# sarahappleby/VAMP

Hardware: AMD Instinct MI355X
Metric: walker-steps/sec (log-posterior evals/sec) (higher is better)
Workload: dtype f64

## Files before the change

### __graft_entry__.py

```python
import os
import subprocess
import sys

ROOT = os.path.dirname(os.path.abspath(__file__))
if ROOT not in sys.path:
    sys.path.insert(0, ROOT)


def build() -> None:
    from vamp_amd import build as vb
    vb.build()
    subprocess.check_call(["make", "-C", os.path.join(ROOT, "oracle"), "-s"])
    host = os.path.join(ROOT, "tests", "host")
    so = os.path.join(host, "libvoigt_host.so")
    src = os.path.join(host, "voigt_host.cpp")
    hdr = os.path.join(ROOT, "vamp_amd", "csrc", "voigt_math.hpp")
    if not os.path.exists(so) or os.path.getmtime(so) < max(os.path.getmtime(src), os.path.getmtime(hdr)):
        subprocess.check_call(["g++", "-O2", "-std=c++17", "-shared", "-fPIC", "-ffp-contract=off", "-o", so, src])
    pso, psrc = os.path.join(host, "libff_pred_host.so"), os.path.join(host, "ff_pred_host.cpp")
    phdr = os.path.join(ROOT, "vamp_amd", "csrc", "ff_predicates.hpp")
    if not os.path.exists(pso) or os.path.getmtime(pso) < max(os.path.getmtime(psrc), os.path.getmtime(phdr), os.path.getmtime(hdr)):
        subprocess.check_call(["g++", "-O2", "-std=c++17", "-shared", "-fPIC", "-ffp-contract=off", "-o", pso, psrc])
    oso, osrc = os.path.join(host, "libnp_order_host.so"), os.path.join(host, "np_order_host.cpp")
    if not os.path.exists(oso) or os.path.getmtime(oso) < max(os.path.getmtime(osrc), os.path.getmtime(phdr), os.path.getmtime(hdr)):
        subprocess.check_call(["g++", "-O2", "-std=c++17", "-shared", "-fPIC", "-ffp-contract=off", "-o", oso, osrc])
    sso, ssrc = os.path.join(host, "libsuper_nodes_host.so"), os.path.join(host, "super_nodes_host.cpp")
    sinc = os.path.join(ROOT, "vamp_amd", "csrc", "ff_super.inc")
    if not os.path.exists(sso) or os.path.getmtime(sso) < max(os.path.getmtime(ssrc), os.path.getmtime(phdr), os.path.getmtime(hdr), os.path.getmtime(sinc)):
        subprocess.check_call(["g++", "-O2", "-std=c++17", "-shared", "-fPIC", "-ffp-contract=off", "-o", sso, ssrc])
    gso, gsrc = os.path.join(host, "libvoigt_grad_host.so"), os.path.join(host, "voigt_grad_host.cpp")
    ghdr = os.path.join(ROOT, "vamp_amd", "csrc", "voigt_grad.hpp")
    if not os.path.exists(gso) or os.path.getmtime(gso) < max(os.path.getmtime(gsrc), os.path.getmtime(ghdr), os.path.getmtime(hdr)):
        subprocess.check_call(["g++", "-O2", "-std=c++17", "-shared", "-fPIC", "-ffp-contract=off", "-o", gso, gsrc])
    fake, fsrc = os.path.join(host, "librccl_fake.so"), os.path.join(host, "rccl_fake.cpp")
    if not os.path.exists(fake) or os.path.getmtime(fake) < os.path.getmtime(fsrc):
        subprocess.check_call([os.environ.get("HIPCC", "/opt/rocm/bin/hipcc"), "-O1", "-std=c++17", "-shared", "-fPIC", "-o", fake, fsrc, "-lrt"])
    import vamp_amd
    os.environ.setdefault("VAMP_NO_IMPORT_ORDER_WARNING", "1")
    vamp_amd._lib.load()


def smoke() -> None:
    import numpy as np
    import torch

    import vamp_amd
    from oracle import vamp_oracle as vo

    g = np.load(os.path.join(ROOT, "tests", "golden", "lnprob_cases.npz"), allow_pickle=False)
    name = "H1215_r0_K4_m1_sd0"
    x, f, n, th = g[name + "_x"], g[name + "_flux"], g[name + "_noise"], g[name + "_theta"]
    region = vo.Region(x=x, flux=f, noise=n, n_comp=4, mode=vo.MODE_VOIGT4)
# ... 44 lines not shown
```

### vamp_amd/csrc/ff_predicates.hpp

```cpp
#pragma once
#include "voigt_math.hpp"

namespace vamp {

constexpr double FF_ZONE_MARGIN = 1.0 / 1024.0;

VAMP_DEV bool ff_tile_in_zone(double c, double s, double y, double mid, double half) {
    const double Xf = (fabs(mid - c) + half) * s;
    return fma(Xf, Xf, y * y) < R2_CORE * (1.0 - FF_ZONE_MARGIN);
}

#ifndef VAMP_SUPER_DIST
#define VAMP_SUPER_DIST 4.0
#endif
#ifndef VAMP_FF_R2_M3
#define VAMP_FF_R2_M3 300.0
#endif
VAMP_DEV bool ff_super_distant(double c, double s, double y, double Mid, double Half) {
    const double distS = fabs(Mid - c) - Half;
    const double Xe = distS * s;
    return (distS >= VAMP_SUPER_DIST * Half) & (fma(Xe, Xe, y * y) >= VAMP_FF_R2_M3);
}
VAMP_DEV double ff_super_r2e(double c, double s, double y, double Mid, double Half) {
    const double Xe = (fabs(Mid - c) - Half) * s;
    return fma(Xe, Xe, y * y);
}
VAMP_DEV void ff_super_tile(double mid0, double half0, double mid3, double half3, double& Mid, double& Half) {
    const double lo = fmin(mid0 - half0, mid3 - half3), hi = fmax(mid0 + half0, mid3 + half3);
    Mid = 0.5 * (lo + hi);
    Half = 0.5 * (hi - lo);
}

struct SuperOrder {
    unsigned long long seq;
    int n, iters, iters3;
};
VAMP_DEV SuperOrder super_order(unsigned dist, unsigned d3) {
    SuperOrder o;
    const unsigned cls[2] = {d3 & dist, dist & ~d3};
    unsigned long long seq = 0ull;
    int sh = 0;
    for (int c = 0; c < 2; ++c)
        for (unsigned m = cls[c]; m; m &= m - 1u) {
            seq |= (unsigned long long)__builtin_ctz(m) << sh;
            sh += 4;
        }
    o.seq = seq;
    o.n = sh >> 2;
    o.iters = (o.n + 7) >> 3;
    o.iters3 = (__builtin_popcount(cls[0]) + 7) >> 3;
    return o;
}

// ... 29 lines not shown
```

### vamp_amd/csrc/vamp_hip.hip

```cpp
#include <hip/hip_runtime.h>
#include <dlfcn.h>

#include <algorithm>
#include <atomic>
#include <chrono>
#include <cmath>
#include <cstdint>
#include <cstdio>
#include <cstdlib>
#include <cstring>
#include <new>
#include <string>
#include <vector>

#include "../../include/vamp_hip.h"
#include "abi_state.hpp"
#include "draws.hpp"
#include "host_plan.hpp"
#include "map_search.hpp"
#include "voigt_math.hpp"
#include "ff_predicates.hpp"
#include "ff_moments.hpp"

#ifndef VAMP_EARLY_LOADS
// ... 50 lines not shown
#ifndef VAMP_MID_Z2
#define VAMP_MID_Z2 30.25
#endif
#ifndef VAMP_WIDE_MAX
#define VAMP_WIDE_MAX 0.75
#endif
#ifndef VAMP_F32_LEAN_STAGE
#define VAMP_F32_LEAN_STAGE 1
#endif
#ifndef VAMP_TILE_MOMENTS
#define VAMP_TILE_MOMENTS 2
#endif
#ifndef VAMP_NODE_PASS
#define VAMP_NODE_PASS 1
#endif
#ifndef VAMP_NP_CLASS_RUNS
#define VAMP_NP_CLASS_RUNS 1
#endif
#ifndef VAMP_DEAL_ADJ
#define VAMP_DEAL_ADJ 1
#endif
#ifndef VAMP_SUPER_NODES
#define VAMP_SUPER_NODES 1
#endif
#ifndef VAMP_TAB_PAIR
#define VAMP_TAB_PAIR 0
#endif
#ifndef VAMP_TILE_HEAD
#define VAMP_TILE_HEAD 0
#endif
namespace {

constexpr int KMAX = 16;
constexpr int KMAX_ALL = VAMP_MAX_COMPONENTS;
static_assert(KMAX_ALL >= KMAX && KMAX_ALL < 64, "lane k stages line k; one spare lane for sd");
constexpr int WAVES_PER_BLOCK = 4;
constexpr long long PACK_MIN_WALKERS = 16384;
constexpr int RES_MAX_MOVERS = 128;
#ifndef VAMP_RES_WAVES
#define VAMP_RES_WAVES 8
#endif
constexpr int RES_MAX_WAVES = VAMP_RES_WAVES;
constexpr int BLOCK = 64 * WAVES_PER_BLOCK;
constexpr int DMAX = 4 * KMAX_ALL + 1;
#ifndef VAMP_SPLIT_MAX_WALKERS
#define VAMP_SPLIT_MAX_WALKERS (1ll << 62)
// ... 956 lines not shown
            chi = fma(r, r, chi);
        }
    }
    }
}

#if VAMP_NODE_PASS && VAMP_TILE_MOMENTS != 1 && !VAMP_X_PREFETCH && !defined(VAMP_SKIP_NEAR) && !defined(VAMP_SKIP_FFNODES) && \
    !defined(VAMP_SKIP_CLENSHAW) && !defined(VAMP_SKIP_EXP)
#define VAMP_NODE_PASS_ON 1
#else
#define VAMP_NODE_PASS_ON 0
#endif
#if VAMP_NODE_PASS_ON
__device__ __forceinline__ unsigned ff_fold16(unsigned long long m) {
    const unsigned h = (unsigned)m | (unsigned)(m >> 32);
    return (h | (h >> 16)) & 0xffffu;
}
#if VAMP_SUPER_NODES && VAMP_DEAL_ADJ
#define VAMP_SUPER_ON 1
#include "ff_super.inc"
#else
#define VAMP_SUPER_ON 0
#endif
struct NodeSets { unsigned far, n6, n4, n3, wide; };
template <bool WIDE, bool ZONE, class LDS>
__device__ __forceinline__ void ff_classify_batch_np(const LDS& L, const double2* __restrict__ geo, int K, int lane_, int base, int stride,
                                                     unsigned wide_all, unsigned long long& farmasks, unsigned long long& widemasks,
                                                     unsigned long long& zonemasks, NodeSets& sets, double& mid, double& half) {
    int lane = lane_;
    asm volatile("" : "+v"(lane));
    const int j = lane >> 4, k = lane & (KMAX - 1);
    const double2 g = geo[(base + j * stride) >> 8];
    mid = g.x, half = fabs(g.y);
    const LineRec& me = *reinterpret_cast<const LineRec*>(reinterpret_cast<const char*>(L.line) +
                                                          __umul24((unsigned)(k < K ? k : 0), (unsigned)sizeof(LineRec)));
    const double my_c = me.c, my_s = me.s, my_y = me.y, my_w8 = me.w8, my_wmid = me.wmid;
    const double dist = fabs(mid - my_c) - half;
    const bool my_beyond = (k < K) & (dist >= FF_DIST * half);
    const bool my_far = my_beyond & (dist >= my_w8);
    const double Xe = dist * my_s, r2e = fma(Xe, Xe, my_y * my_y);
    farmasks = __ballot(my_far);
    sets.far = ff_fold16(farmasks);
    sets.n6 = ff_fold16(__ballot(my_far & (r2e < VAMP_FF_R2_M4)));
    sets.n4 = ff_fold16(__ballot(my_far & (r2e < VAMP_FF_R2_M3)));
    sets.n3 = ff_fold16(__ballot(my_far & (r2e < VAMP_FF_R2_M2)));
    widemasks = 0ull;
    if constexpr (WIDE) {
        const bool my_wide = ((((wide_all >> k) & 1u) != 0u) | (VAMP_MID_NODES && (my_beyond & (dist >= my_wmid)))) & !my_far;
        widemasks = __ballot(my_wide);
    }
    sets.wide = ff_fold16(widemasks);
    zonemasks = 0ull;
    if constexpr (ZONE) zonemasks = __ballot(vamp::ff_tile_in_zone(my_c, my_s, my_y, mid, half));
}
constexpr double FF_X_IDLE = 64.0;
static_assert(FF_X_IDLE * FF_X_IDLE >= VAMP_FF_R2_M2 && FF_X_IDLE < vamp::X_FAR, "the idle argument neither deepens a pair nor needs a guard");
template <int M> struct NpDepth { static constexpr int value = M; };
#if VAMP_SUPER_ON
template <class LDS>
__device__ __forceinline__ double ff_super_pass(const LDS& L, TileScratch& Sx, const double* __restrict__ dct, int lane, double xnode,
                                                unsigned dist, unsigned d3, double Mid, double Half) {
    const vamp::SuperOrder ord = vamp::super_order(dist, d3);
    const int n = lane & (FF_NODES - 1), g4 = (lane >> 4) * 4;
    const double xs = fma(Half, dct[FF_MAT + n], Mid);
    unsigned long long seq = ord.seq;
    int left = ord.n;
    double acc = 0.0;
    auto run = [&](auto depth, int iters) {
        constexpr int M = decltype(depth)::value;
#pragma unroll 1
        for (int i = 0; i < iters; ++i) {
            const unsigned s32 = (unsigned)seq >> g4;
            double X[2], y[2], amp[2], r2[2], nn[2], d[2];
#pragma unroll
            for (int t = 0; t < 2; ++t) {
                const LineRec& ln = *reinterpret_cast<const LineRec*>(reinterpret_cast<const char*>(L.line) +
                                                                      __umul24((s32 >> (16 * t)) & 15u, (unsigned)sizeof(LineRec)));
                const bool live = (g4 >> 2) + 4 * t < left;
                const double Xl = fabs(xs - ln.c) * ln.s;
                X[t] = live ? Xl : FF_X_IDLE;
                y[t] = ln.y;
                amp[t] = live ? ln.amp : 0.0;
                r2[t] = fma(X[t], X[t], y[t] * y[t]);
                vamp::voigt_jfrac_nd<M>(X[t], y[t], r2[t], nn[t], d[t], vamp::GHFrac<M>::Z, vamp::GHFrac<M>::C);
            }
            const double ra = vamp::rcp_nr(d[0] * d[1]);
            acc = fma(amp[0], nn[0] * (ra * d[1]), acc);
            acc = fma(amp[1], nn[1] * (ra * d[0]), acc);
            seq >>= 32;
            left -= 8;
        }
    };
    run(NpDepth<3>{}, ord.iters3);
    run(NpDepth<2>{}, ord.iters - ord.iters3);
    {
        const int me = lane_here();
        const int a16 = (me ^ 16) << 2, a32 = (me ^ 32) << 2;
        acc += __hiloint2double(__builtin_amdgcn_ds_bpermute(a16, __double2hiint(acc)), __builtin_amdgcn_ds_bpermute(a16, __double2loint(acc)));
        acc += __hiloint2double(__builtin_amdgcn_ds_bpermute(a32, __double2hiint(acc)), __builtin_amdgcn_ds_bpermute(a32, __double2loint(acc)));
    }
    if (lane < FF_NODES) Sx.coef[lane] = acc;
    __builtin_amdgcn_wave_barrier();
    const double2* crow = reinterpret_cast<const double2*>(FF_SUPER_C) + n;
    const double2* fv = reinterpret_cast<const double2*>(Sx.coef);
    double a0 = 0.0, a1 = 0.0;
#pragma unroll
    for (int n2 = 0; n2 < FF_NODES / 2; ++n2) {
        const double2 m = crow[n2 * FF_NODES], f2 = fv[n2];
        a0 = fma(m.x, f2.x, a0);
        a1 = fma(m.y, f2.y, a1);
    }
    __builtin_amdgcn_wave_barrier();
    if (lane < FF_NODES) Sx.coef[lane] = a0 + a1;
    __builtin_amdgcn_wave_barrier();
    const double t = (xnode - Mid) * vamp::rcp_nr(Half), t2 = t + t;
    double b1 = 0.0, b2 = 0.0;
#pragma unroll
    for (int k = FF_NODES - 1; k >= 1; --k) {
        const double b = fma(t2, b1, Sx.coef[k] - b2);
        b2 = b1;
        b1 = b;
    }
    const double p = fma(t, b1, Sx.coef[0] - b2);
    __builtin_amdgcn_wave_barrier();
    return p;
}
template <class LDS>
__device__ __forceinline__ double ff_super_batch(const LDS& L, TileScratch& Sx, const double* __restrict__ dct, const double2* __restrict__ geo,
                                                 int K, int lane_, int base, int stride, double mid, double half,
                                                 unsigned long long farmasks, NodeSets& sets) {
    int lane = lane_;
    asm volatile("" : "+v"(lane));
    const int k = lane & (KMAX - 1);
    const LineRec& me = *reinterpret_cast<const LineRec*>(reinterpret_cast<const char*>(L.line) +
                                                          __umul24((unsigned)(k < K ? k : 0), (unsigned)sizeof(LineRec)));
    const double my_c = me.c, my_s = me.s, my_y = me.y;
    const double2 g0 = geo[base >> 8], g3 = geo[(base + (FF_BATCH - 1) * stride) >> 8];
    double Mid, Half;
    vamp::ff_super_tile(g0.x, fabs(g0.y), g3.x, fabs(g3.y), Mid, Half);
    const bool my_dist = (k < K) & vamp::ff_super_distant(my_c, my_s, my_y, Mid, Half);
    const bool my_d3 = my_dist & (vamp::ff_super_r2e(my_c, my_s, my_y, Mid, Half) < VAMP_FF_R2_M2);
    const unsigned all4 = (unsigned)farmasks & (unsigned)(farmasks >> 16) & (unsigned)(farmasks >> 32) & (unsigned)(farmasks >> 48) & 0xffffu;
    const unsigned dist = (unsigned)__ballot(my_dist) & all4;
    if (dist == 0u) return 0.0;
    const unsigned d3 = (unsigned)__ballot(my_d3) & dist;
    sets.far &= ~dist, sets.n6 &= ~dist, sets.n4 &= ~dist, sets.n3 &= ~dist;
    const double xnode = fma(half, dct[FF_MAT + (lane & (FF_NODES - 1))], mid);
    return ff_super_pass(L, Sx, dct, lane, xnode, dist, d3, Mid, Half);
}
#endif
template <bool WIDE, bool GUARD, class LDS>
__device__ __forceinline__ double ff_node_pass(const LDS& L, const double* __restrict__ dct, const double* tab, int lane_, double mid, double half,
                                               unsigned long long farmasks, unsigned long long widemasks, NodeSets sets, double fs0 = 0.0) {
    int lane = lane_;
    asm volatile("" : "+v"(lane));
    const double xnode = fma(half, dct[FF_MAT + (lane & (FF_NODES - 1))], mid);
    double fs = fs0;
    const unsigned far16 = ff_tile_field(farmasks, lane);
#if VAMP_NP_CLASS_RUNS
    if (sets.far != 0u) {
    const vamp::NpOrder ord = vamp::np_pair_order(sets.far, sets.n6, sets.n4, sets.n3);
    unsigned long long seq = ord.seq;
    const unsigned far16b = far16 & ~ord.solo;
    struct Pair { double c[2], s[2], y[2], amp[2]; };
    auto read_pair = [&](unsigned long long q) {
        Pair p;
#pragma unroll
        for (int t = 0; t < 2; ++t) {
            const LineRec& ln = L.line[(unsigned)(q >> (4 * t)) & 15u];
            p.c[t] = ln.c, p.s[t] = ln.s, p.y[t] = ln.y, p.amp[t] = ln.amp;
        }
// ... 123 lines not shown
}
__device__ __forceinline__ void ff_moment_chi_nodes_row(TileScratch& Sx, const double* __restrict__ mt, int lane, int j, double a_row, double c0,
                                                        double& chi) {
    if ((lane >> 4) == j) Sx.coef[lane & (FF_NODES - 1)] = a_row;
    const int n = lane & (FF_NODES - 1), g4 = (lane >> 4) * 4;
    const double2* Qr = reinterpret_cast<const double2*>(mt + vamp::FFN_Q + n * FF_NODES + g4);
    const double2 q01 = Qr[0], q23 = Qr[1];
    const double Sv = mt[vamp::FFN_S + n];
    __builtin_amdgcn_wave_barrier();
    const double2* av = reinterpret_cast<const double2*>(Sx.coef + g4);
    const double2 a01 = av[0], a23 = av[1];
    const double a = Sx.coef[n];
    const double acc0 = fma(q01.x, a01.x, 0.5 * Sv), acc1 = q01.y * a01.y;
    const double term = a * (fma(q23.x, a23.x, acc0) + fma(q23.y, a23.y, acc1));
    chi += lane == 0 ? term + c0 : term;
    __builtin_amdgcn_wave_barrier();
}
template <int MODE, class PK, bool TAB, bool WIDE = false, bool GUARD = true, bool SUPER = false>
__device__ __forceinline__ void sweep_range_ff_np(const RegionDev& R, const typename PK::Lds& L, TileScratch& Sx, const double* __restrict__ dct,
                                                  const double* __restrict__ x, const double* __restrict__ f,
                                                  const double* __restrict__ wt, const double* __restrict__ ut,
                                                  const double2* __restrict__ geo, int lane, int base0, int base1, int stride,
                                                  double& chi, const double* tab, unsigned long long wide_all = 0ull,
                                                  const double* __restrict__ mom = nullptr) {
    constexpr int T = TPIX;
    static_assert(PK::LPW == 64 && PK::KCAP <= 16, "far-field tiles: one walker per wavefront, <= 16 lines");
    const int K = R.K;
    const int ntile = base0 < base1 ? (base1 - base0 + stride - 1) / stride : 0;
#if VAMP_DEAL_ADJ
    (void)ntile;
    const int tstride = 64 * T, bstep = FF_BATCH * stride;
    const int bfull = __builtin_amdgcn_readfirstlane((base1 / bstep) * bstep);
    const int bfirst = FF_BATCH * base0, brest = bfull + base0;
#else
    const int tstride = stride, bstep = FF_BATCH * stride;
    const int bfull = __builtin_amdgcn_readfirstlane(base0 + (ntile / FF_BATCH) * (FF_BATCH * stride));
    const int bfirst = base0, brest = bfull;
#endif
    for (int batch = __builtin_amdgcn_readfirstlane(bfirst); batch < bfull; batch += bstep) {
    unsigned long long farmasks, widemasks, zonemasks;
    double fsn;
    {
        NodeSets sets;
        double mid_j, half_j;
        ff_classify_batch_np<WIDE, TAB>(L, geo, K, lane, batch, tstride, (unsigned)wide_all, farmasks, widemasks, zonemasks, sets, mid_j, half_j);
#if VAMP_SUPER_ON
        double fs0 = 0.0;
        if constexpr (SUPER) {
            if (__builtin_amdgcn_readfirstlane((int)(unsigned)wide_all) == 0) {
                fs0 = ff_super_batch(L, Sx, dct, geo, K, lane, batch, tstride, mid_j, half_j, farmasks, sets);
            }
        }
        fsn = ff_node_pass<WIDE, GUARD>(L, dct, tab, lane, mid_j, half_j, farmasks, widemasks, sets, fs0);
#else
        fsn = ff_node_pass<WIDE, GUARD>(L, dct, tab, lane, mid_j, half_j, farmasks, widemasks, sets);
#endif
    }
#if VAMP_TILE_MOMENTS == 2
    {
        unsigned long long fm = farmasks, wm = widemasks;
        double a_row = 0.0, amax_row = 0.0;
        bool have_a = false;
#pragma unroll 1
        for (int j = 0; j < FF_BATCH; ++j, fm >>= KMAX, wm >>= KMAX) {
            const unsigned farmask = (unsigned)fm & 0xffffu, widemask = WIDE ? (unsigned)wm & 0xffffu : 0u;
            if ((~(farmask | widemask) & ((1u << K) - 1u)) != 0u) continue;
            const double* mt = mom + ((batch + j * tstride) >> 8) * MOM_TILE;
            const double root_c0 = mt[MOM_RC], root_q0 = mt[MOM_RQ];
            if (!vamp::ff_moments_try(root_c0, root_q0)) continue;
            if (!have_a) {
                int eoff = FF_EXP;
                asm volatile("" : "+s"(eoff));
                a_row = -vamp::expm1_taylor_tab(-fsn, dct + eoff);
// ... 314 lines not shown
#endif
#ifndef VAMP_SKIP_CLENSHAW
            ff32_horner<T>(Sx, u, up, tau);
#endif
        }
#pragma unroll
        for (int t = 0; t < T; ++t) {
            const int i = base + 64 * t + lane;
#ifdef VAMP_SKIP_EXP
            const float m = 1.0f - tau[t];
#else
            const float m = __expf(-tau[t]);
#endif
            const float r = (f[i] - m) * wt[i];
            chi += (double)r * (double)r;
        }
    }
    }
}

struct PixPtrs {
    const double* x; const double* f; const double* wt;
    const float* xf; const float* ff; const float* wtf;
    const double* u; const float* uf; const double2* geo;
    const double* mom;
};

template <bool F32>
__global__ __launch_bounds__(64 * TPIX) void k_tile_tables(const RegionDev* __restrict__ regions, const double* __restrict__ x,
                                                           const float* __restrict__ xf, double* __restrict__ u, float* __restrict__ uf,
                                                           double2* __restrict__ geo, const double* __restrict__ f = nullptr,
                                                           const double* __restrict__ wt = nullptr, double* __restrict__ mom = nullptr) {
    const RegionDev& R = regions[blockIdx.y];
    const int base = (int)blockIdx.x * (64 * TPIX), i = base + (int)threadIdx.x;
    if (i >= R.P) return;
    const long long g = R.pix_off + i;
    if (base + 64 * TPIX > R.P) {
        if constexpr (F32) uf[g] = 0.0f;
        else u[g] = 0.0;
        return;
    }
    const long long g0 = R.pix_off + base, g1 = g0 + 64 * TPIX - 1;
    const double x_lo = F32 ? (double)xf[g0] : x[g0], x_hi = F32 ? (double)xf[g1] : x[g1];
    const double mid = 0.5 * (x_lo + x_hi), half = 0.5 * fabs(x_hi - x_lo);
    const bool up = x_hi > x_lo;
    const int t = (int)threadIdx.x >> 6, q = up ? t : TPIX - 1 - t;
    double ug = 0.0;
    if constexpr (F32) {
        const float hf = (float)half, mf = (float)mid;
// ... 99 lines not shown
        if constexpr (VAMP_FARFIELD && PK::FF && MODE != VAMP_GAUSS3 && TPIX == 4)
            sweep_range_f32_ff<MODE, PK, use_tables32<F32, MODE, PK>()>(R, L, Sx, dct, x, f, wt, px.uf + R.pix_off, px.geo + (R.pix_off >> 8),
                                                                        lane, base0, full, stride, chi, reinterpret_cast<const float*>(tab));
        else if (TPIX > 1) sweep_range_f32<MODE, PK, TPIX>(R, L, x, f, wt, lane, base0, full, stride, chi);
        if constexpr (PK::TAIL || TPIX == 1)
            if (tail) {
                const int from = TPIX > 1 ? full : 0;
                if constexpr (!PK::FF && TPIX > 1) {
                    const int nt = (R.P - from + PK::LPW - 1) / PK::LPW;
                    if constexpr (TPIX >= 4) { if (nt == 4) sweep_range_f32<MODE, PK, 4>(R, L, x, f, wt, lane, from, from + 1, 1 << 28, chi); }
                    if constexpr (TPIX >= 3) { if (nt == 3) sweep_range_f32<MODE, PK, 3>(R, L, x, f, wt, lane, from, from + 1, 1 << 28, chi); }
                    if (nt == 2) sweep_range_f32<MODE, PK, 2>(R, L, x, f, wt, lane, from, from + 1, 1 << 28, chi);
                    else if (nt == 1) sweep_range_f32<MODE, PK, 1>(R, L, x, f, wt, lane, from, from + 1, 1 << 28, chi);
                } else {
                    sweep_range_f32<MODE, PK, 1>(R, L, x, f, wt, lane, from, R.P, PK::LPW, chi);
                }
            }
    } else {
        const double* x = px.x + R.pix_off; const double* f = px.f + R.pix_off; const double* wt = px.wt + R.pix_off;
        if constexpr (VAMP_FARFIELD && PK::FF && MODE != VAMP_GAUSS3 && TPIX == 4) {
            const double* ut = px.u + R.pix_off;
            const double2* geo = px.geo + (R.pix_off >> 8);
            const double* mom = VAMP_TILE_MOMENTS ? px.mom + (R.pix_off >> 8) * MOM_TILE : nullptr;
            const int flags = __builtin_amdgcn_readfirstlane((int)(__double_as_longlong(L.theta[4 * PK::KCAP + 2]) & 0x3ffff));
            const bool guard = (flags >> 16) != 0;
            if constexpr (VAMP_WIDE_NODES && TAB) {
                const unsigned long long wide_all = (unsigned long long)(flags & 0xffff);
                if (VAMP_MID_NODES || wide_all) {
                    if (guard) sweep_range_ff_any<MODE, PK, TAB, true, true>(R, L, Sx, dct, x, f, wt, ut, geo, lane, base0, full, stride, chi, tab, wide_all, mom);
                    else sweep_range_ff_any<MODE, PK, TAB, true, false, true>(R, L, Sx, dct, x, f, wt, ut, geo, lane, base0, full, stride, chi, tab, wide_all, mom);
                } else {
                    if (guard) sweep_range_ff_any<MODE, PK, TAB, false, true>(R, L, Sx, dct, x, f, wt, ut, geo, lane, base0, full, stride, chi, tab, 0ull, mom);
                    else sweep_range_ff_any<MODE, PK, TAB, false, false, true>(R, L, Sx, dct, x, f, wt, ut, geo, lane, base0, full, stride, chi, tab, 0ull, mom);
                }
            } else {
                if (guard) sweep_range_ff_any<MODE, PK, TAB, false, true>(R, L, Sx, dct, x, f, wt, ut, geo, lane, base0, full, stride, chi, tab, 0ull, mom);
                else sweep_range_ff_any<MODE, PK, TAB, false, false, true>(R, L, Sx, dct, x, f, wt, ut, geo, lane, base0, full, stride, chi, tab, 0ull, mom);
            }
        } else if (TPIX > 1) sweep_range<MODE, PK, TPIX, TAB>(R, L, x, f, wt, lane, base0, full, stride, chi, tab);
        if constexpr (PK::TAIL || TPIX == 1)
            if (tail) {
                const int from = TPIX > 1 ? full : 0;
                if constexpr (!PK::FF && TPIX > 1) {
                    const int nt = (R.P - from + PK::LPW - 1) / PK::LPW;
                    if constexpr (TPIX >= 4) { if (nt == 4) sweep_range<MODE, PK, 4, TAB>(R, L, x, f, wt, lane, from, from + 1, 1 << 28, chi, tab); }
                    if constexpr (TPIX >= 3) { if (nt == 3) sweep_range<MODE, PK, 3, TAB>(R, L, x, f, wt, lane, from, from + 1, 1 << 28, chi, tab); }
                    if (nt == 2) sweep_range<MODE, PK, 2, TAB>(R, L, x, f, wt, lane, from, from + 1, 1 << 28, chi, tab);
                    else if (nt == 1) sweep_range<MODE, PK, 1, TAB>(R, L, x, f, wt, lane, from, from + 1, 1 << 28, chi, tab);
                } else {
                    sweep_range<MODE, PK, 1, TAB>(R, L, x, f, wt, lane, from, R.P, PK::LPW, chi, tab);
                }
            }
    }
}

template <int MODE, class PK, int T>
__device__ __forceinline__ void blend_chunk(const RegionDev& R, const typename PK::Lds& L, const double* __restrict__ x, int lane,
                                            int base, int k0, int kn, const double* tab, double (&tau)[4]) {
    double xi[T];
#pragma unroll
    for (int t = 0; t < T; ++t) {
// ... 256 lines not shown
    if (!(lp > NEG_INF)) return;
    TileScratch& Sx = scr[wave];
    const double* tab = tabs[0].a;
    const double2* geo = px.geo + (R.pix_off >> 8);
    const int flags = __builtin_amdgcn_readfirstlane((int)(__double_as_longlong(L.theta[4 * PK::KCAP + 2]) & 0x3ffff));
    const bool guard = (flags >> 16) != 0;
    const unsigned wide_all = (unsigned)(flags & 0xffff);
    constexpr int TILE = 64 * TPIX;
    const int K = R.K, base1 = (R.P / TILE) * TILE, stride = PARTS * TILE;
    const int base0 = __builtin_amdgcn_readfirstlane(wave * TILE);
    int bfull = base0, brest = base0;
#if VAMP_NODE_PASS_ON
    const int ntile = base0 < base1 ? (base1 - base0 + stride - 1) / stride : 0;
    const int tstride = adj ? TILE : stride, bstep = FF_BATCH * stride;
    bfull = __builtin_amdgcn_readfirstlane(adj ? (base1 / bstep) * bstep : base0 + (ntile / FF_BATCH) * bstep);
    brest = adj ? bfull + base0 : bfull;
    for (int batch = adj ? FF_BATCH * base0 : base0; batch < bfull; batch += bstep) {
        unsigned long long farmasks, widemasks, zonemasks;
        NodeSets sets;
        double mid, half;
        ff_classify_batch_np<true, true>(L, geo, K, lane, batch, tstride, wide_all, farmasks, widemasks, zonemasks, sets, mid, half);
        double fs0 = 0.0;
#if VAMP_SUPER_ON
        if (adj && !guard && wide_all == 0u) fs0 = ff_super_batch(L, Sx, dct, geo, K, lane, batch, tstride, mid, half, farmasks, sets);
#endif
        const double fs = guard ? ff_node_pass<true, true>(L, dct, tab, lane, mid, half, farmasks, widemasks, sets)
                                : ff_node_pass<true, false>(L, dct, tab, lane, mid, half, farmasks, widemasks, sets, fs0);
        nodes[((batch + (lane >> 4) * tstride) >> 8) * FF_NODES + (lane & (FF_NODES - 1))] = fs;
        if (lane == 0) {
            unsigned* so = sets_out + (batch >> 8) * 5;
            so[0] = sets.far, so[1] = sets.n6, so[2] = sets.n4, so[3] = sets.n3, so[4] = sets.wide;
        }
    }
#endif
    for (int batch = brest; batch < base1; batch += FF_BATCH * stride) {
        unsigned long long farmasks, widemasks, zonemasks;
        ff_classify_batch<true, false, true>(L, Sx, geo, K, lane, batch, base1, stride, wide_all, farmasks, widemasks, zonemasks);
        for (int j = 0; j < FF_BATCH; ++j, farmasks >>= KMAX, widemasks >>= KMAX) {
            const int base = batch + j * stride;
            if (base >= base1) break;
            const double2 tg = geo[base >> 8];
            const double mid = tg.x, half = fabs(tg.y);
            const int nfar = __builtin_popcount((unsigned)farmasks & 0xffffu), nwide = __builtin_popcount((unsigned)widemasks & 0xffffu);
            const double fs_wide = nwide > 0 ? ff_wide_nodes<typename PK::Lds>(L, Sx.widelist[j], dct, tab, lane, nwide, mid, half) : 0.0;
            const double fs = guard ? ff_node_sums<typename PK::Lds, true>(L, Sx.farlist[j], dct, lane, nfar, mid, half, fs_wide)
                                    : ff_node_sums<typename PK::Lds, false>(L, Sx.farlist[j], dct, lane, nfar, mid, half, fs_wide);
            if (lane < FF_NODES) nodes[(base >> 8) * FF_NODES + lane] = fs;
// ... 666 lines not shown
    DevBuf<long long> nacc_d;
    DevBuf<double> send_d;
    DevBuf<double> recv_d;
    void* rccl = nullptr;
    hipStream_t comm_stream = nullptr;
    std::vector<hipEvent_t> ev_kernel, ev_scatter;
    EventPairs xtiming;
    DevBuf<double> sc_th, sc_lp, sc_chi;
    PinnedBuf<double> pin_th, pin_out;
    DevBuf<double> map_th_d, map_best_d, map_sim_d;
    DevBuf<unsigned char> map_act_d;
    DevBuf<long long> map_it_d;
    int opt_map_device = 1;
    int opt_resident = 1;
    DevBuf<int> ext_act_d, ext_par_d;
    DevBuf<double> ext_z_d, ext_lu_d;
    bool timing = false;
    EventPairs ktiming;

    DevBuf<double> u_d;
    DevBuf<float> uf_d;
    DevBuf<double2> geo_d;
    DevBuf<double> mom_d;

    PixPtrs pix() const {
        return PixPtrs{x_d.get(), f_d.get(), wt_d.get(), xf_d.get(), ff_d.get(), wtf_d.get(), u_d.get(), uf_d.get(), geo_d.get(), mom_d.get()};
    }
};

namespace {

void reset_regions(vamp_ctx* c) {
    c->regions_d.reset();
    c->x_d.reset(); c->f_d.reset(); c->wt_d.reset();
    c->xf_d.reset(); c->ff_d.reset(); c->wtf_d.reset();
    c->u_d.reset(); c->uf_d.reset(); c->geo_d.reset(); c->mom_d.reset();
    c->classes.clear();
    c->classes_small.clear();
    c->n_regions = 0;
}

void reset_sampler(vamp_ctx* c) {
    c->X_own.reset(); c->lnp_own.reset();
    c->X_d = c->lnp_d = nullptr;
    c->nacc_d.reset();
    c->send_d.reset(); c->recv_d.reset();
    c->exchange = false;
    c->sampler_ready = false;
}

int ensure_part_events(vamp_ctx* c, int parts);
int alloc_exchange_buffers(vamp_ctx* c) {
    HIP_TRY(c->send_d.ensure(vamp::exchange_send_doubles(c)));
    HIP_TRY(c->recv_d.ensure(vamp::exchange_recv_doubles(c)));
    vamp::exchange_parts(c);
    c->exchange = true;
    if (c->comm) return ensure_part_events(c, c->shard_parts);
    return 0;
}
// ... 463 lines not shown
            row[1] = shape;
            row[2] = shape_walkers_per_block(shape);
            row[3] = shape_threads(shape);
            row[4] = (long long)cl.regions.size();
        }
        ++n;
    }
    return n;
}

long long vampdbg_tile_tables(vamp_ctx* c, double* u_out, float* uf_out, double* geo_out) {
    if (!c || !geo_out || !(c->f32 ? (void*)uf_out : (void*)u_out)) return fail(VAMP_ERR_ARG, "vampdbg_tile_tables: bad argument");
    if (c->regions_h.empty()) return fail(VAMP_ERR_STATE, "vampdbg_tile_tables: call vamp_set_regions first");
    if (!c->geo_d) return 0;
    const long long N = c->regions_h.back().pix_off + c->regions_h.back().P;
    const long long slots = N / (64 * TPIX) + 1;
    HIP_TRY(hipStreamSynchronize(c->stream));
    if (c->f32) HIP_TRY(hipMemcpy(uf_out, c->uf_d.get(), N * sizeof(float), hipMemcpyDeviceToHost));
    else HIP_TRY(hipMemcpy(u_out, c->u_d.get(), N * sizeof(double), hipMemcpyDeviceToHost));
    HIP_TRY(hipMemcpy(geo_out, c->geo_d.get(), slots * sizeof(double2), hipMemcpyDeviceToHost));
    return slots;
}

long long vampdbg_tile_moments(vamp_ctx* c, double* out) {
    if (!c) return fail(VAMP_ERR_ARG, "vampdbg_tile_moments: bad argument");
    if (c->regions_h.empty()) return fail(VAMP_ERR_STATE, "vampdbg_tile_moments: call vamp_set_regions first");
    if (!VAMP_TILE_MOMENTS || c->f32 || !c->geo_d || !c->mom_d) return 0;
    const long long N = c->regions_h.back().pix_off + c->regions_h.back().P;
    const long long slots = N / (64 * TPIX) + 1;
    HIP_TRY(hipStreamSynchronize(c->stream));
    if (out) HIP_TRY(hipMemcpy(out, c->mom_d.get(), slots * MOM_TILE * sizeof(double), hipMemcpyDeviceToHost));
    return MOM_TILE;
}

static long long dbg_node_sums(vamp_ctx* c, int region, const double* theta, double* nodes, unsigned* sets, bool adj) {
    if (!c || !theta || !nodes || !sets) return fail(VAMP_ERR_ARG, "vampdbg_node_sums: bad argument");
    if (c->regions_h.empty()) return fail(VAMP_ERR_STATE, "vampdbg_node_sums: call vamp_set_regions first");
    if (region < 0 || region >= c->n_regions) return fail(VAMP_ERR_ARG, "vampdbg_node_sums: no such region");
    const RegionDev& R = c->regions_h[region];
    const long long tiles = R.P / (64 * TPIX);
    if (c->f32 || c->mode == VAMP_GAUSS3 || !c->geo_d || tiles == 0 || R.K > KMAX) return 0;
    HIP_TRY(hipSetDevice(c->device));
    DevBuf<double> th_d, nodes_d;
    DevBuf<unsigned> sets_d;
    HIP_TRY(th_d.ensure(R.D));
    HIP_TRY(nodes_d.ensure(tiles * FF_NODES));
// ... 118 lines not shown
    const long long N = pix_off[n_regions];
    const std::vector<double> wt = vamp::pixel_weights(N, noise, sample_sd);
    HIP_TRY(c->x_d.ensure(N));
    HIP_TRY(c->f_d.ensure(N));
    HIP_TRY(c->wt_d.ensure(N));
    HIP_TRY(hipMemcpy(c->x_d.get(), x, N * sizeof(double), hipMemcpyHostToDevice));
    HIP_TRY(hipMemcpy(c->f_d.get(), flux, N * sizeof(double), hipMemcpyHostToDevice));
    HIP_TRY(hipMemcpy(c->wt_d.get(), wt.data(), N * sizeof(double), hipMemcpyHostToDevice));
    if (c->f32) {
        std::vector<float> t(N);
        HIP_TRY(c->xf_d.ensure(N));
        HIP_TRY(c->ff_d.ensure(N));
        HIP_TRY(c->wtf_d.ensure(N));
        for (long long i = 0; i < N; ++i) t[i] = (float)x[i];
        HIP_TRY(hipMemcpy(c->xf_d.get(), t.data(), N * sizeof(float), hipMemcpyHostToDevice));
        for (long long i = 0; i < N; ++i) t[i] = (float)flux[i];
        HIP_TRY(hipMemcpy(c->ff_d.get(), t.data(), N * sizeof(float), hipMemcpyHostToDevice));
        for (long long i = 0; i < N; ++i) t[i] = (float)wt[i];
        HIP_TRY(hipMemcpy(c->wtf_d.get(), t.data(), N * sizeof(float), hipMemcpyHostToDevice));
    }
    HIP_TRY(c->regions_d.ensure(n_regions));
    HIP_TRY(hipMemcpy(c->regions_d.get(), R.data(), n_regions * sizeof(RegionDev), hipMemcpyHostToDevice));
    int max_tiles = 0;
    bool any_full = false;
    for (const RegionDev& d : R) {
        max_tiles = std::max(max_tiles, (d.P + 64 * TPIX - 1) / (64 * TPIX));
        any_full = any_full || d.P >= 64 * TPIX;
    }
    if (mode != VAMP_GAUSS3 && any_full) {
        if (c->f32) HIP_TRY(c->uf_d.ensure(N));
        else HIP_TRY(c->u_d.ensure(N));
        HIP_TRY(c->geo_d.ensure(N / (64 * TPIX) + 1));
        if (VAMP_TILE_MOMENTS && !c->f32) {
            HIP_TRY(c->mom_d.ensure((N / (64 * TPIX) + 1) * MOM_TILE));
            HIP_TRY(hipMemsetAsync(c->mom_d.get(), 0, (N / (64 * TPIX) + 1) * MOM_TILE * sizeof(double), c->stream));
        }
        VAMP_FOR_F32(c->f32, hipLaunchKernelGGL((k_tile_tables<F32>), dim3((unsigned)max_tiles, (unsigned)n_regions), dim3(64 * TPIX), 0,
                                                c->stream, c->regions_d.get(), c->x_d.get(), c->xf_d.get(), c->u_d.get(),
                                                c->uf_d.get(), c->geo_d.get(), c->f_d.get(), c->wt_d.get(), c->mom_d.get()));
        HIP_TRY(hipGetLastError());
        HIP_TRY(hipStreamSynchronize(c->stream));
    }
    for (int which = 0; which < 2; ++which) {
        const vamp::plan::ClassPlan& pl = which ? c->plan_small : c->plan;
        std::vector<LaunchClass>& part = which ? c->classes_small : c->classes;
        for (size_t k = 0; k < pl.kind.size(); ++k) part.push_back(LaunchClass{pl.kind[k], pl.regions[k]});
#if VAMP_LPT
        bool reordered = false;
        if (which == 1 || VAMP_LPT == 2)
            for (LaunchClass& cl : part) {
                std::vector<int> before = cl.regions;
                std::stable_sort(cl.regions.begin(), cl.regions.end(), [&](int a, int b) {
                    return (long long)R[a].K * R[a].P > (long long)R[b].K * R[b].P;
                });
                reordered = reordered || before != cl.regions;
            }
        if (part.size() > 1 || reordered)
#else
        if (part.size() > 1)
#endif
            for (LaunchClass& cl : part) {
                HIP_TRY(cl.list_d.ensure(cl.regions.size()));
                HIP_TRY(hipMemcpy(cl.list_d.get(), cl.regions.data(), cl.regions.size() * sizeof(int), hipMemcpyHostToDevice));
// ... 500 lines not shown
```

Baseline: 15.24 million.

## Precompute per-batch super-tile barycentric interpolation weights at region setup

Adds a setup kernel that computes, for each far-field batch, the barycentric interpolation weights mapping super-tile Chebyshev nodes to each sub-tile's nodes. These weights are stored in a device buffer. The super pass then reads the weights and does a 16-term dot product instead of the per-lane Chebyshev/Clenshaw evaluation against the coefficient matrix. This trades per-evaluation arithmetic for extra global memory reads of 64*16 doubles per batch and an extra device buffer. The weights depend only on fixed pixel geometry, not on walker parameters.

```diff
diff --git a/__graft_entry__.py b/__graft_entry__.py
--- a/__graft_entry__.py
+++ b/__graft_entry__.py
@@ -28,6 +28,9 @@
     sinc = os.path.join(ROOT, "vamp_amd", "csrc", "ff_super.inc")
     if not os.path.exists(sso) or os.path.getmtime(sso) < max(os.path.getmtime(ssrc), os.path.getmtime(phdr), os.path.getmtime(hdr), os.path.getmtime(sinc)):
         subprocess.check_call(["g++", "-O2", "-std=c++17", "-shared", "-fPIC", "-ffp-contract=off", "-o", sso, ssrc])
+    iso, isrc = os.path.join(host, "libsuper_interp_host.so"), os.path.join(host, "super_interp_host.cpp")
+    if not os.path.exists(iso) or os.path.getmtime(iso) < max(os.path.getmtime(isrc), os.path.getmtime(phdr), os.path.getmtime(hdr)):
+        subprocess.check_call(["g++", "-O2", "-std=c++17", "-shared", "-fPIC", "-ffp-contract=off", "-o", iso, isrc])
     gso, gsrc = os.path.join(host, "libvoigt_grad_host.so"), os.path.join(host, "voigt_grad_host.cpp")
     ghdr = os.path.join(ROOT, "vamp_amd", "csrc", "voigt_grad.hpp")
     if not os.path.exists(gso) or os.path.getmtime(gso) < max(os.path.getmtime(gsrc), os.path.getmtime(ghdr), os.path.getmtime(hdr)):
diff --git a/vamp_amd/csrc/ff_predicates.hpp b/vamp_amd/csrc/ff_predicates.hpp
--- a/vamp_amd/csrc/ff_predicates.hpp
+++ b/vamp_amd/csrc/ff_predicates.hpp
@@ -29,6 +29,20 @@
     const double lo = fmin(mid0 - half0, mid3 - half3), hi = fmax(mid0 + half0, mid3 + half3);
     Mid = 0.5 * (lo + hi);
     Half = 0.5 * (hi - lo);
+}
+VAMP_DEV double ff_super_row(double mid, double half, double node, double Mid, double Half, const double* tn, double* w) {
+    const double xnode = fma(half, node, mid);
+    const double t = (xnode - Mid) / Half;
+    double den = 0.0;
+    int hit = -1;
+    for (int m = 0; m < 16; ++m) {
+        const double tm = tn[m], bm = sqrt((1.0 - tm) * (1.0 + tm)), diff = t - tm;
+        if (diff == 0.0) hit = m;
+        w[m] = ((m & 1) ? -bm : bm) / diff;
+        den += w[m];
+    }
+    for (int m = 0; m < 16; ++m) w[m] = hit < 0 ? w[m] / den : (m == hit ? 1.0 : 0.0);
+    return t;
 }
 
 struct SuperOrder {
diff --git a/vamp_amd/csrc/vamp_hip.hip b/vamp_amd/csrc/vamp_hip.hip
--- a/vamp_amd/csrc/vamp_hip.hip
+++ b/vamp_amd/csrc/vamp_hip.hip
@@ -96,6 +96,9 @@
 #endif
 #ifndef VAMP_SUPER_NODES
 #define VAMP_SUPER_NODES 1
+#endif
+#ifndef VAMP_SUPER_INTERP
+#define VAMP_SUPER_INTERP 1
 #endif
 #ifndef VAMP_TAB_PAIR
 #define VAMP_TAB_PAIR 0
@@ -1098,6 +1101,8 @@
 #else
 #define VAMP_SUPER_ON 0
 #endif
+#define VAMP_SUPER_INTERP_ON (VAMP_SUPER_ON && VAMP_SUPER_INTERP)
+constexpr int SUPER_REC = 64 * FF_NODES;
 struct NodeSets { unsigned far, n6, n4, n3, wide; };
 template <bool WIDE, bool ZONE, class LDS>
 __device__ __forceinline__ void ff_classify_batch_np(const LDS& L, const double2* __restrict__ geo, int K, int lane_, int base, int stride,
@@ -1134,7 +1139,12 @@
 template <int M> struct NpDepth { static constexpr int value = M; };
 #if VAMP_SUPER_ON
 template <class LDS>
-__device__ __forceinline__ double ff_super_pass(const LDS& L, TileScratch& Sx, const double* __restrict__ dct, int lane, double xnode,
+__device__ __forceinline__ double ff_super_pass(const LDS& L, TileScratch& Sx, const double* __restrict__ dct, int lane,
+#if VAMP_SUPER_INTERP_ON
+                                                const double* __restrict__ rec,
+#else
+                                                double xnode,
+#endif
                                                 unsigned dist, unsigned d3, double Mid, double Half) {
     const vamp::SuperOrder ord = vamp::super_order(dist, d3);
     const int n = lane & (FF_NODES - 1), g4 = (lane >> 4) * 4;
@@ -1169,6 +1179,14 @@
     };
     run(NpDepth<3>{}, ord.iters3);
     run(NpDepth<2>{}, ord.iters - ord.iters3);
+#if VAMP_SUPER_INTERP_ON
+    double2 w[FF_NODES / 2];
+    {
+        const double2* wrow = reinterpret_cast<const double2*>(rec) + lane_here();
+#pragma unroll
+        for (int n2 = 0; n2 < FF_NODES / 2; ++n2) w[n2] = wrow[n2 * 64];
+    }
+#endif
     {
         const int me = lane_here();
         const int a16 = (me ^ 16) << 2, a32 = (me ^ 32) << 2;
@@ -1177,6 +1195,19 @@
     }
     if (lane < FF_NODES) Sx.coef[lane] = acc;
     __builtin_amdgcn_wave_barrier();
+#if VAMP_SUPER_INTERP_ON
+    const double2* fv = reinterpret_cast<const double2*>(Sx.coef);
+    double a0 = 0.0, a1 = 0.0;
+#pragma unroll
+    for (int n2 = 0; n2 < FF_NODES / 2; ++n2) {
+        const double2 f2 = fv[n2];
+        a0 = fma(w[n2].x, f2.x, a0);
+        a1 = fma(w[n2].y, f2.y, a1);
+    }
+    const double p = a0 + a1;
+    __builtin_amdgcn_wave_barrier();
+    return p;
+#else
     const double2* crow = reinterpret_cast<const double2*>(FF_SUPER_C) + n;
     const double2* fv = reinterpret_cast<const double2*>(Sx.coef);
     double a0 = 0.0, a1 = 0.0;
@@ -1200,11 +1231,16 @@
     const double p = fma(t, b1, Sx.coef[0] - b2);
     __builtin_amdgcn_wave_barrier();
     return p;
+#endif
 }
 template <class LDS>
 __device__ __forceinline__ double ff_super_batch(const LDS& L, TileScratch& Sx, const double* __restrict__ dct, const double2* __restrict__ geo,
                                                  int K, int lane_, int base, int stride, double mid, double half,
-                                                 unsigned long long farmasks, NodeSets& sets) {
+                                                 unsigned long long farmasks, NodeSets& sets
+#if VAMP_SUPER_INTERP_ON
+                                                 , const double* __restrict__ sup
+#endif
+                                                 ) {
     int lane = lane_;
     asm volatile("" : "+v"(lane));
     const int k = lane & (KMAX - 1);
@@ -1221,8 +1257,13 @@
     if (dist == 0u) return 0.0;
     const unsigned d3 = (unsigned)__ballot(my_d3) & dist;
     sets.far &= ~dist, sets.n6 &= ~dist, sets.n4 &= ~dist, sets.n3 &= ~dist;
+#if VAMP_SUPER_INTERP_ON
+    (void)mid, (void)half;
+    return ff_super_pass(L, Sx, dct, lane, sup + (size_t)(base >> 8) * SUPER_REC, dist, d3, Mid, Half);
+#else
     const double xnode = fma(half, dct[FF_MAT + (lane & (FF_NODES - 1))], mid);
     return ff_super_pass(L, Sx, dct, lane, xnode, dist, d3, Mid, Half);
+#endif
 }
 #endif
 template <bool WIDE, bool GUARD, class LDS>
@@ -1392,7 +1433,11 @@
                                                   const double* __restrict__ wt, const double* __restrict__ ut,
                                                   const double2* __restrict__ geo, int lane, int base0, int base1, int stride,
                                                   double& chi, const double* tab, unsigned long long wide_all = 0ull,
-                                                  const double* __restrict__ mom = nullptr) {
+                                                  const double* __restrict__ mom = nullptr
+#if VAMP_SUPER_INTERP_ON
+                                                  , const double* __restrict__ sup = nullptr
+#endif
+                                                  ) {
     constexpr int T = TPIX;
     static_assert(PK::LPW == 64 && PK::KCAP <= 16, "far-field tiles: one walker per wavefront, <= 16 lines");
     const int K = R.K;
@@ -1418,7 +1463,11 @@
         double fs0 = 0.0;
         if constexpr (SUPER) {
             if (__builtin_amdgcn_readfirstlane((int)(unsigned)wide_all) == 0) {
+#if VAMP_SUPER_INTERP_ON
+                fs0 = ff_super_batch(L, Sx, dct, geo, K, lane, batch, tstride, mid_j, half_j, farmasks, sets, sup);
+#else
                 fs0 = ff_super_batch(L, Sx, dct, geo, K, lane, batch, tstride, mid_j, half_j, farmasks, sets);
+#endif
             }
         }
         fsn = ff_node_pass<WIDE, GUARD>(L, dct, tab, lane, mid_j, half_j, farmasks, widemasks, sets, fs0);
@@ -1779,9 +1828,33 @@
 struct PixPtrs {
     const double* x; const double* f; const double* wt;
     const float* xf; const float* ff; const float* wtf;
+#if VAMP_SUPER_INTERP_ON
+    const double* u; union { const float* uf; const double* sup; }; const double2* geo;
+#else
     const double* u; const float* uf; const double2* geo;
+#endif
     const double* mom;
 };
+
+#if VAMP_SUPER_INTERP_ON
+__global__ __launch_bounds__(64) void k_super_records(const RegionDev* __restrict__ regions, const double2* __restrict__ geo,
+                                                      double* __restrict__ sup) {
+    const RegionDev& R = regions[blockIdx.y];
+    constexpr int TILE = 64 * TPIX;
+    const int base = (int)blockIdx.x * (FF_BATCH * TILE);
+    if (base + FF_BATCH * TILE > R.P) return;
+    const int lane = (int)threadIdx.x, j = lane >> 4, n = lane & (FF_NODES - 1);
+    const long long s0 = (R.pix_off >> 8) + (base >> 8);
+    const double2 g = geo[s0 + j], g0 = geo[s0], g3 = geo[s0 + FF_BATCH - 1];
+    double Mid, Half;
+    vamp::ff_super_tile(g0.x, fabs(g0.y), g3.x, fabs(g3.y), Mid, Half);
+    double w[FF_NODES];
+    vamp::ff_super_row(g.x, fabs(g.y), FF_M[FF_MAT + n], Mid, Half, FF_M + FF_MAT, w);
+    double* rec = sup + s0 * SUPER_REC;
+#pragma unroll
+    for (int m = 0; m < FF_NODES; ++m) rec[(m >> 1) * 128 + 2 * lane + (m & 1)] = w[m];
+}
+#endif
 
 template <bool F32>
 __global__ __launch_bounds__(64 * TPIX) void k_tile_tables(const RegionDev* __restrict__ regions, const double* __restrict__ x,
@@ -1927,21 +2000,28 @@
             const double* ut = px.u + R.pix_off;
             const double2* geo = px.geo + (R.pix_off >> 8);
             const double* mom = VAMP_TILE_MOMENTS ? px.mom + (R.pix_off >> 8) * MOM_TILE : nullptr;
+#if VAMP_SUPER_INTERP_ON
+            const double* sup = px.sup + (size_t)(R.pix_off >> 8) * SUPER_REC;
+#define VAMP_SUP_ARG , sup
+#else
+#define VAMP_SUP_ARG
+#endif
             const int flags = __builtin_amdgcn_readfirstlane((int)(__double_as_longlong(L.theta[4 * PK::KCAP + 2]) & 0x3ffff));
             const bool guard = (flags >> 16) != 0;
             if constexpr (VAMP_WIDE_NODES && TAB) {
                 const unsigned long long wide_all = (unsigned long long)(flags & 0xffff);
                 if (VAMP_MID_NODES || wide_all) {
                     if (guard) sweep_range_ff_any<MODE, PK, TAB, true, true>(R, L, Sx, dct, x, f, wt, ut, geo, lane, base0, full, stride, chi, tab, wide_all, mom);
-                    else sweep_range_ff_any<MODE, PK, TAB, true, false, true>(R, L, Sx, dct, x, f, wt, ut, geo, lane, base0, full, stride, chi, tab, wide_all, mom);
+                    else sweep_range_ff_any<MODE, PK, TAB, true, false, true>(R, L, Sx, dct, x, f, wt, ut, geo, lane, base0, full, stride, chi, tab, wide_all, mom VAMP_SUP_ARG);
                 } else {
                     if (guard) sweep_range_ff_any<MODE, PK, TAB, false, true>(R, L, Sx, dct, x, f, wt, ut, geo, lane, base0, full, stride, chi, tab, 0ull, mom);
-                    else sweep_range_ff_any<MODE, PK, TAB, false, false, true>(R, L, Sx, dct, x, f, wt, ut, geo, lane, base0, full, stride, chi, tab, 0ull, mom);
+                    else sweep_range_ff_any<MODE, PK, TAB, false, false, true>(R, L, Sx, dct, x, f, wt, ut, geo, lane, base0, full, stride, chi, tab, 0ull, mom VAMP_SUP_ARG);
                 }
             } else {
                 if (guard) sweep_range_ff_any<MODE, PK, TAB, false, true>(R, L, Sx, dct, x, f, wt, ut, geo, lane, base0, full, stride, chi, tab, 0ull, mom);
-                else sweep_range_ff_any<MODE, PK, TAB, false, false, true>(R, L, Sx, dct, x, f, wt, ut, geo, lane, base0, full, stride, chi, tab, 0ull, mom);
+                else sweep_range_ff_any<MODE, PK, TAB, false, false, true>(R, L, Sx, dct, x, f, wt, ut, geo, lane, base0, full, stride, chi, tab, 0ull, mom VAMP_SUP_ARG);
             }
+#undef VAMP_SUP_ARG
         } else if (TPIX > 1) sweep_range<MODE, PK, TPIX, TAB>(R, L, x, f, wt, lane, base0, full, stride, chi, tab);
         if constexpr (PK::TAIL || TPIX == 1)
             if (tail) {
@@ -2244,7 +2324,12 @@
         ff_classify_batch_np<true, true>(L, geo, K, lane, batch, tstride, wide_all, farmasks, widemasks, zonemasks, sets, mid, half);
         double fs0 = 0.0;
 #if VAMP_SUPER_ON
+#if VAMP_SUPER_INTERP_ON
+        if (adj && !guard && wide_all == 0u)
+            fs0 = ff_super_batch(L, Sx, dct, geo, K, lane, batch, tstride, mid, half, farmasks, sets, px.sup + (size_t)(R.pix_off >> 8) * SUPER_REC);
+#else
         if (adj && !guard && wide_all == 0u) fs0 = ff_super_batch(L, Sx, dct, geo, K, lane, batch, tstride, mid, half, farmasks, sets);
+#endif
 #endif
         const double fs = guard ? ff_node_pass<true, true>(L, dct, tab, lane, mid, half, farmasks, widemasks, sets)
                                 : ff_node_pass<true, false>(L, dct, tab, lane, mid, half, farmasks, widemasks, sets, fs0);
@@ -2957,9 +3042,16 @@
     DevBuf<float> uf_d;
     DevBuf<double2> geo_d;
     DevBuf<double> mom_d;
+    DevBuf<double> sup_d;
 
     PixPtrs pix() const {
+#if VAMP_SUPER_INTERP_ON
+        PixPtrs p{x_d.get(), f_d.get(), wt_d.get(), xf_d.get(), ff_d.get(), wtf_d.get(), u_d.get(), {uf_d.get()}, geo_d.get(), mom_d.get()};
+        if (!f32) p.sup = sup_d.get();
+        return p;
+#else
         return PixPtrs{x_d.get(), f_d.get(), wt_d.get(), xf_d.get(), ff_d.get(), wtf_d.get(), u_d.get(), uf_d.get(), geo_d.get(), mom_d.get()};
+#endif
     }
 };
 
@@ -2969,7 +3061,7 @@
     c->regions_d.reset();
     c->x_d.reset(); c->f_d.reset(); c->wt_d.reset();
     c->xf_d.reset(); c->ff_d.reset(); c->wtf_d.reset();
-    c->u_d.reset(); c->uf_d.reset(); c->geo_d.reset(); c->mom_d.reset();
+    c->u_d.reset(); c->uf_d.reset(); c->geo_d.reset(); c->mom_d.reset(); c->sup_d.reset();
     c->classes.clear();
     c->classes_small.clear();
     c->n_regions = 0;
@@ -3479,6 +3571,22 @@
     return slots;
 }
 
+long long vampdbg_super_records(vamp_ctx* c, double* out) {
+    if (!c) return fail(VAMP_ERR_ARG, "vampdbg_super_records: bad argument");
+    if (c->regions_h.empty()) return fail(VAMP_ERR_STATE, "vampdbg_super_records: call vamp_set_regions first");
+#if VAMP_SUPER_INTERP_ON
+    if (c->f32 || !c->geo_d || !c->sup_d) return 0;
+    const long long N = c->regions_h.back().pix_off + c->regions_h.back().P;
+    const long long slots = N / (64 * TPIX) + 1;
+    HIP_TRY(hipStreamSynchronize(c->stream));
+    if (out) HIP_TRY(hipMemcpy(out, c->sup_d.get(), slots * SUPER_REC * sizeof(double), hipMemcpyDeviceToHost));
+    return SUPER_REC;
+#else
+    (void)out;
+    return 0;
+#endif
+}
+
 long long vampdbg_tile_moments(vamp_ctx* c, double* out) {
     if (!c) return fail(VAMP_ERR_ARG, "vampdbg_tile_moments: bad argument");
     if (c->regions_h.empty()) return fail(VAMP_ERR_STATE, "vampdbg_tile_moments: call vamp_set_regions first");
@@ -3643,11 +3751,13 @@
     HIP_TRY(c->regions_d.ensure(n_regions));
     HIP_TRY(hipMemcpy(c->regions_d.get(), R.data(), n_regions * sizeof(RegionDev), hipMemcpyHostToDevice));
     int max_tiles = 0;
-    bool any_full = false;
+    bool any_full = false, any_batch = false;
     for (const RegionDev& d : R) {
         max_tiles = std::max(max_tiles, (d.P + 64 * TPIX - 1) / (64 * TPIX));
         any_full = any_full || d.P >= 64 * TPIX;
-    }
+        any_batch = any_batch || d.P >= FF_BATCH * 64 * TPIX;
+    }
+    (void)any_batch;
     if (mode != VAMP_GAUSS3 && any_full) {
         if (c->f32) HIP_TRY(c->uf_d.ensure(N));
         else HIP_TRY(c->u_d.ensure(N));
@@ -3660,6 +3770,16 @@
                                                 c->stream, c->regions_d.get(), c->x_d.get(), c->xf_d.get(), c->u_d.get(),
                                                 c->uf_d.get(), c->geo_d.get(), c->f_d.get(), c->wt_d.get(), c->mom_d.get()));
         HIP_TRY(hipGetLastError());
+#if VAMP_SUPER_INTERP_ON
+        if (!c->f32 && any_batch) {
+            const size_t sup_n = (size_t)(N / (64 * TPIX) + 1) * SUPER_REC;
+            HIP_TRY(c->sup_d.ensure(sup_n));
+            HIP_TRY(hipMemsetAsync(c->sup_d.get(), 0, sup_n * sizeof(double), c->stream));
+            hipLaunchKernelGGL(k_super_records, dim3((unsigned)(max_tiles / FF_BATCH), (unsigned)n_regions), dim3(64), 0, c->stream,
+                               c->regions_d.get(), c->geo_d.get(), c->sup_d.get());
+            HIP_TRY(hipGetLastError());
+        }
+#endif
         HIP_TRY(hipStreamSynchronize(c->stream));
     }
     for (int which = 0; which < 2; ++which) {
```

After: 15.30 million, median of 6. About the same (+0.4%).
